# gabormarko/3D-semantic-segmentation

Hardware: AMD Instinct MI355X
Metric: Mvoxel-views/sec (higher is better)
Workload: dtype f32; 1 GPU; R2: 200000 voxels x 300 views x 968x548x512 fp32 feature maps, room-shell scene seed 0, dmin 0.01 dmax 10 step 0.5*voxel; views_per_call=60, resident_feature_maps=60, parallelism=single GPU

## Files before the change

3d-semantic-segmentation_amd/csrc/voxproj.hip:

```cpp
#include <hip/hip_runtime.h>

#include <cmath>
#include <cstdarg>
#include <cstdint>
#include <cstdio>
#include <cstdlib>
#include <cstring>
#include <algorithm>
#include <chrono>
#include <mutex>
#include <unordered_map>
#include <vector>

#include "voxproj.h"

#include "vp_common.h"
#include "vp_tables.h"
#include "vp_march.h"
#include "vp_gather.h"
#include "vp_aux.h"
#include "vp_prep.h"
#include "vp_aggregate.h"
#include "vp_render.h"
#include "vp_query.h"
// ... 199 lines not shown
        long long ppx = rec.opt_part_px > 0 ? rec.opt_part_px : std::max<long long>(1, heavy_t);
        ppx = std::max(ppx, (px2 + l.slot_cap - 1) / l.slot_cap);
        plan.part_px = (int)std::min<long long>(ppx, 2147483647ll);
        heavy_t = std::max(heavy_t, plan.part_px);
        plan.heavy_t = plan.part_t = heavy_t;
    } else if (one_split) {
        const long long T = rec.opt_one_view_split > 0 ? rec.opt_one_view_split : rec.opt_heavy_t > 0 ? rec.opt_heavy_t : 0;
        long long ppx = rec.opt_part_px > 0 ? std::max(rec.opt_part_px, (px2 + l.slot_cap - 1) / l.slot_cap) : 0;
        if (ppx == 0 && T > 0) ppx = std::max<long long>((T + ONE_VIEW_T_RATIO - 1) / ONE_VIEW_T_RATIO, (px2 + l.slot_cap - 1) / l.slot_cap);
        plan.part_px = (int)std::min<long long>(ppx, 2147483646ll);
        plan.dyn_px_min = ppx > 0 ? 0 : ONE_VIEW_PART_MIN;
        plan.heavy_t = plan.part_t = T > 0 ? (int)std::min<long long>(std::max(T, ppx), 2147483646ll) : 0;
        plan.dyn_t_ratio = T > 0 ? 0 : ONE_VIEW_T_RATIO;
        plan.dyn_t_floor = (long long)H * W <= GATHER_G32_SMALL_IMAGE ? ONE_VIEW_T_FLOOR_SMALL : 0;
        plan.cell_in_item = 1;
        heavy_t = plan.heavy_t;
    } else if (one_view) {
        plan.count_heavy = 0;
    }
    static_assert(sizeof(PlanArgs) == sizeof(int) * 8, "PlanArgs is kept as ints in the workspace record");
    if (gather_only) { memcpy(&plan, st->last_plan, sizeof(plan)); heavy_t = plan.heavy_t; }
    const int part_px = plan.part_px;
    const bool plans_parts = part_px > 0 || plan.dyn_px_min > 0;
#ifdef VP_DIAG
    if (flags & VP_FLAG_DIAG_EVALS) heavy_t = -1;
    if (flags & VP_FLAG_DIAG_WAVES) heavy_t = -2;
#endif
    const int wl_blocks = (int)((n_rows + 256 * WL_PER_THREAD - 1) / (256 * WL_PER_THREAD));
    int4 *parts = (int4 *)(ws + l.parts[q]), *split = (int4 *)(ws + l.split[q]), *pmeta = (int4 *)(ws + l.pmeta[q]);
    float *prow = (float *)(ws + l.prow[q]);
    int *hit_waves = (int *)(ws + l.hitcnt[q]);
#define VP_LAUNCH_WORKLIST(STREAM)                                                                                              \
    hipLaunchKernelGGL(k_worklist, dim3((unsigned)(wl_blocks + (B * V + 255) / 256)), dim3(256), 0, STREAM, (const int *)cnt_call,   \
                       plan, (long long)n_rows, work, status, wl_blocks, vmi, viewtab, B * V, row_lo, row_hi, parts, split, \
                       (int)l.slot_cap, rec.sticky_dev, (const int *)cell_of_id, (const int *)hit_waves, (int)l.n_hitcnt)
    if (gather_only) {
        VP_HIP(hipMemsetAsync(status + ST_WORK0, 0, ST_PLAN_WORDS * sizeof(int), s0));
        VP_LAUNCH_WORKLIST(s0);
    }
    if (!gather_only) {
        ProfSpan sp; sp.begin(0, s1);
        hipLaunchKernelGGL(k_zero_call, dim3((unsigned)((n_rows + 1023) / 1024)), dim3(256), 0, s1, status, cnt_call, (long long)n_rows,
                           status0, rec.sticky_dev, WS_MAGIC, rec.gen, expect_tables, hit_waves,
                           (plan.dyn_px_min > 0 && !march_only) ? l.n_hitcnt : 0ll);
        sp.end();
    }
    if (!gather_only) {
        FirstHitArgs fa;
        fa.occ = (const long long *)occ; fa.vmi = vmi; fa.intr = intr; fa.near2 = near2; fa.dist = dist;
        fa.nby = l.nby; fa.nbx = l.nbx; fa.nblk = l.nblk; fa.hit = march_only ? (int *)ids_out : hit; fa.cnt_call = cnt_call;
        fa.heavy_list = heavy_list; fa.heavy_t = ((one_view && !one_split) || heavy_t < 0) ? heavy_t : 2147483647;
        fa.hit_waves = (plan.dyn_px_min > 0 && l.n_hitcnt > 0) ? hit_waves : nullptr;
        if (march_only) { fa.heavy_t = 2147483647; fa.hit_waves = nullptr; }
        fa.status = status; fa.sticky = rec.sticky_dev;
        const dim3 grid((W + 15) / 16, (H + 15) / 16, B * V);
        ProfSpan sp; sp.begin(1, s1);
        if (flags & VP_FLAG_EXACT_MARCH) {
            hipLaunchKernelGGL(k_first_hit<0>, grid, dim3(256), 0, s1, fa, p);
        } else {
            bool beside_gather = false;
            if (pipe && ps->used[q ^ 1]) {
                beside_gather = hipEventQuery(ps->call_done[q ^ 1]) == hipErrorNotReady;
                (void)hipGetLastError();
            }
            const size_t row_bytes = size_t(C) * (feats_f16 ? 2 : 4);
            size_t lds_req = beside_gather ? (row_bytes <= 1024 ? 30 : 41) * 1024 : 0;
            if (rec.opt_march_lds_kb >= 0) lds_req = size_t(std::min<long long>(rec.opt_march_lds_kb, 64)) * 1024;
            hipLaunchKernelGGL(k_first_hit<1>, grid, dim3(256), lds_req, s1, fa, p);
        }
        if (!march_only) VP_LAUNCH_WORKLIST(s1);
        sp.end();
    }
    if (march_only) {
        VP_HIP(hipGetLastError());
        ps->last_q = 0;
        if (flags & VP_FLAG_SYNC) return workspace_status_impl(workspace, stream_, true);
        return VP_OK;
    }
    if (pipe && !gather_only) VP_HIP(hipEventRecord(ps->fh_done[q], s1));

    GatherArgs g;
    g.feats = feats; g.hit = hit; g.viewtab = viewtab; g.intr = intr; g.cell_of_id = cell_of_id;
    g.cnt_call = cnt_call; g.heavy_list = heavy_list; g.n_heavy = status + ST_NHEAVY;
    g.row_lo = (int)row_lo; g.row_hi = (int)row_hi;
    g.work = work; g.work_n = status + ST_WORK0;
    g.parts = parts; g.split = split; g.pmeta = pmeta; g.prow = prow;
    g.host_word = nullptr; g.host_seq = 0;
    g.parts_on = (one_view && plans_parts) ? 1 : 0; g.slot_cap = (int)l.slot_cap; g.count = count; g.views_hit = views_hit; g.out = out; g.status = status;
    const int vec_ok = feats_f16 ? 2 : ((C % 4 == 0) && (((uintptr_t)feats & 15) == 0) && (((uintptr_t)out & 15) == 0)) ? 1 : 0;
    const bool small_image = (long long)B * V >= 8 && (long long)H * W <= GATHER_G32_SMALL_IMAGE;
    g.heavy_blocks = 0;
    if (pipe && !gather_only) VP_HIP(hipStreamWaitEvent(s0, ps->fh_done[q], 0));
    if (one_view) {
        ProfSpan sp; sp.begin(2, s0);
        const int per_cu = rec.opt_one_view > 0 ? (int)std::min<long long>(rec.opt_one_view, 256) : 16;
        const long long want = rec.opt_one_view >= 1000 ? rec.opt_one_view - 1000 : (long long)device_cus() * per_cu;
        const long long cap = (n_rows - 1 + 3) / 4;
        const unsigned nblk = (unsigned)std::max<long long>(1, std::min(want, cap));
        g.heavy_blocks = (heavy_t != 2147483647 && !plans_parts) ? (int)nblk : 0;
        volatile int *note = nullptr;
        if ((flags & VP_FLAG_SYNC) && plans_parts && n_rows > 1) {
            rec.split_seq = (rec.split_seq + 1) & 0x7fffu;
            note = rec.sticky_host + ST_HOST_NSPLIT;
            *note = 0;
            g.host_word = rec.sticky_dev + ST_HOST_NSPLIT; g.host_seq = (int)rec.split_seq;
        }
        if (n_rows > 1) VP_DISPATCH_GATHER_ONE((long long)H * W <= GATHER_G32_SMALL_IMAGE, vec_ok, C, dim3(nblk), dim3(256), 0, s0, g, p);
        sp.end();
        bool combine = n_rows > 1 && plans_parts;
        if (combine && note) {
            const auto t0 = std::chrono::steady_clock::now();
            for (unsigned spin = 0;; spin++) {
                const unsigned v = (unsigned)*note;
                if ((v >> 31) && ((v >> 16) & 0x7fffu) == rec.split_seq) { combine = (v & 0xffffu) != 0; break; }
                if ((spin & 63) == 63 && std::chrono::steady_clock::now() - t0 > std::chrono::milliseconds(2)) break;
                __builtin_ia32_pause();
            }
        }
        if (combine) {
            ProfSpan sc; sc.begin(3, s0);
// ... 820 lines not shown
    if (radius > 0)
        if (int rc = eval_check_workspace(workspace, workspace_bytes, W, H)) return rc;
    hipStream_t stream = (hipStream_t)stream_;
    const long long n = (long long)W * H;
    unsigned char *pband = nullptr, *tband = nullptr;
    if (radius > 0) {
        const size_t plane = align256((size_t)n);
        pband = (unsigned char *)workspace;
        tband = pband + plane;
        unsigned char *ok = tband + plane;
        eval_launch_band((const int *)pred, W, H, radius, pband, ok, stream);
        eval_launch_band((const int *)target, W, H, radius, tband, ok, stream);
    }
    const dim3 grid((unsigned)std::min<long long>((n + 255) / 256, EVAL_SCORE_BLOCKS));
#define VP_EVAL_SCORES(LDS) hipLaunchKernelGGL((k_eval_scores<LDS>), grid, dim3(256), 0, stream, (const int *)pred, (const int *)target, n, \
        P, (const unsigned char *)pband, (const unsigned char *)tband, (unsigned long long *)confusion,                              \
        (unsigned long long *)skipped, (unsigned long long *)bnd_inter, (unsigned long long *)bnd_union)
    if (P <= EVAL_LDS_P) VP_EVAL_SCORES(true); else VP_EVAL_SCORES(false);
#undef VP_EVAL_SCORES
    VP_HIP(hipGetLastError());
    return VP_OK;
}

long long vp_workspace_table_builds(const void *workspace)
{
    WsState *rec = ws_state(workspace, false);
    return rec ? rec->builds : 0;
}

int vp_workspace_create(void *workspace, size_t workspace_bytes)
{
    if (!workspace) return fail(VP_EINVAL, "null workspace");
    if ((uintptr_t)workspace & 255) return fail(VP_EWORKSPACE, "workspace must be 256-byte aligned");
    if (workspace_bytes < 2 * align256(ST_WORDS * sizeof(int))) return fail(VP_EWORKSPACE, "workspace has %zu bytes, need at least %zu", workspace_bytes, 2 * align256(ST_WORDS * sizeof(int)));
    ws_forget(workspace);
    (void)ws_state(workspace, true);
    return VP_OK;
}

int vp_workspace_set_option(void *workspace, int option, long long value)
{
    if (!workspace) return fail(VP_EINVAL, "null workspace");
    WsState *rec = ws_state(workspace, true);
    switch (option) {
    case VP_OPT_HEAVY_THRESHOLD: rec->opt_heavy_t = value > 0 ? value : -1; return VP_OK;
    case VP_OPT_MARCH_LDS_KB:
        if (value > 64) return fail(VP_EINVAL, "VP_OPT_MARCH_LDS_KB = %lld: the march's dynamic-LDS reservation is limited to 64 KiB (0 .. 64; < 0 = default)", value);
        rec->opt_march_lds_kb = value >= 0 ? value : -1; return VP_OK;
    case VP_OPT_ROW_BEGIN:       rec->opt_row_begin = value >= 0 ? value : -1; return VP_OK;
    case VP_OPT_ROW_END:         rec->opt_row_end = value >= 0 ? value : -1; return VP_OK;
    case VP_OPT_ONE_VIEW_GATHER: rec->opt_one_view = value >= 0 ? value : -1; return VP_OK;
    case VP_OPT_PART_PIXELS:     rec->opt_part_px = value > 0 ? value : -1; return VP_OK;
    case VP_OPT_ONE_VIEW_SPLIT:  rec->opt_one_view_split = value >= 0 ? value : -1; return VP_OK;
    default: return fail(VP_EINVAL, "unknown workspace option %d", option);
    }
}

int vp_workspace_release(void *workspace)
{
    ws_forget(workspace);
    return VP_OK;
}

}
```

3d-semantic-segmentation_amd/csrc/vp_common.h:

```cpp
#pragma once

namespace {

thread_local char g_err[512] = "";

int fail(int code, const char *fmt, ...)
{
    va_list ap;
    va_start(ap, fmt);
    vsnprintf(g_err, sizeof(g_err), fmt, ap);
    va_end(ap);
    return code;
}

#define VP_HIP(call)                                                                      \
    do {                                                                                  \
        hipError_t e_ = (call);                                                           \
        if (e_ != hipSuccess)                                                             \
            return fail(VP_EHIP, "%s failed: %s (%s:%d)", #call, hipGetErrorString(e_),   \
                        __FILE__, __LINE__);                                              \
    } while (0)

struct Profile {
    std::mutex mu;
// ... 6 lines not shown
        if (used * 2 == pool.size()) {
            hipEvent_t e0, e1;
            if (hipEventCreate(&e0) != hipSuccess || hipEventCreate(&e1) != hipSuccess) return -1;
            pool.push_back(e0); pool.push_back(e1); kind.push_back(0);
        }
        kind[used] = k;
        return (int)used++;
    }
} g_prof;

struct ProfSpan {
    int idx = -1;
    hipStream_t stream = nullptr;
    void begin(int k, hipStream_t s)
    {
        std::lock_guard<std::mutex> g(g_prof.mu);
        if (!g_prof.on) return;
        idx = g_prof.next(k);
        stream = s;
        if (idx >= 0) (void)hipEventRecord(g_prof.pool[idx * 2], s);
    }
    void end()
    {
        if (idx < 0) return;
        std::lock_guard<std::mutex> g(g_prof.mu);
        (void)hipEventRecord(g_prof.pool[idx * 2 + 1], stream);
        idx = -1;
    }
};

struct PipeState {
    hipStream_t side = nullptr;
    hipEvent_t fh_done[2] = {nullptr, nullptr};
    hipEvent_t call_done[2] = {nullptr, nullptr};
    bool used[2] = {false, false};
    long long calls = 0;
    int last_q = 0;
    bool ok = false;
};
struct WsState {
    unsigned gen = 0;
    int B = 0, dimz = 0, dimy = 0, dimx = 0;
    long long n_rows = 0;
    bool copy_valid = false;
    long long builds = 0;
    bool opened = false;
    int *sticky_host = nullptr, *sticky_dev = nullptr;
    long long opt_heavy_t = -1;
    long long opt_march_lds_kb = -1;
    long long opt_row_begin = -1, opt_row_end = -1;
    long long opt_one_view = -1;
    long long opt_part_px = -1;
    long long opt_one_view_split = -1;
    int last_B = 0, last_V = 0, last_H = 0, last_W = 0, last_C = 0, last_q = 0;
    bool last_f16 = false, last_ranged = false;
    int last_plan[8] = {0, 0, 0, 0, 0, 0, 0, 0};
    unsigned split_seq = 0;
    const void *last_feats = nullptr, *last_out = nullptr, *last_count = nullptr, *last_vmi = nullptr;
    bool has_hit = false;
    size_t hit_off = 0;
    PipeState pipe;
};
std::mutex g_ws_mu;
std::unordered_map<const void *, WsState *> g_ws;
unsigned g_next_gen = 0;

WsState *ws_state(const void *workspace, bool create)
{
    std::lock_guard<std::mutex> g(g_ws_mu);
    auto it = g_ws.find(workspace);
    if (it != g_ws.end()) return it->second;
    if (!create) return nullptr;
    if (g_next_gen == 0) g_next_gen = (unsigned)std::chrono::steady_clock::now().time_since_epoch().count() | 1u;
    WsState *st = new WsState();
    st->gen = g_next_gen;
    g_next_gen += 2;
    g_ws.emplace(workspace, st);
    return st;
}

void pipe_destroy(PipeState &ps)
{
    if (!ps.ok) return;
    (void)hipStreamSynchronize(ps.side);
    (void)hipStreamDestroy(ps.side);
    for (int q = 0; q < 2; q++) {
        (void)hipEventDestroy(ps.fh_done[q]);
        (void)hipEventDestroy(ps.call_done[q]);
    }
    ps = PipeState();
}

void ws_forget(const void *workspace)
{
    WsState *st = nullptr;
    {
        std::lock_guard<std::mutex> g(g_ws_mu);
        auto it = g_ws.find(workspace);
        if (it == g_ws.end()) return;
        st = it->second;
        g_ws.erase(it);
    }
    pipe_destroy(st->pipe);
    if (st->sticky_host) (void)hipHostFree(st->sticky_host);
    delete st;
}
// ... 42 lines not shown
    int width, height;
    float dmin, dmax, inc;
    float ox, oy, oz, vs;
    int dimz, dimy, dimx;
    int B, V, C;
    long long n_rows;
};

enum { ST_BADID = 0, ST_BOXMISS = 1, ST_NHEAVY = 2, ST_ZERO = 3 , ST_STUCK = 4, ST_OCCDIFF = 5, ST_STALE = 6,
       ST_HEAVY_T = 7,
       ST_NHIT = 8,
       ST_PART_T = 9, ST_PART_PX = 10,
       ST_WORK0 = 16, WORK_CLASSES = 8,
       ST_NPARTS = 24, ST_NSPLIT = 25,
       ST_PLAN_WORDS = WORK_CLASSES + 2,
       ST_CALL_WORDS = 32,
       ST_HDR_MAGIC = 56, ST_HDR_GEN = 57, ST_HDR_TABLES = 58,
       ST_HOST_NSPLIT = 60,
       ST_STICKY_STALE = 61, ST_STICKY_BADID = 62, ST_STICKY_STUCK = 63, ST_WORDS = 64 };
constexpr unsigned WS_MAGIC = 0x56585033u;
#ifdef VP_DIAG
enum { VP_FLAG_DIAG_EVALS = 1 << 20,
       VP_FLAG_DIAG_WAVES = 1 << 21 };
#endif

inline unsigned tables_key(int B, int dimz, int dimy, int dimx, long long n_rows, long long builds)
{
    unsigned long long h = 0x9E3779B97F4A7C15ull;
    const long long v[6] = {B, dimz, dimy, dimx, n_rows, builds};
    for (long long x : v) { h ^= (unsigned long long)x + 0x9E3779B97F4A7C15ull + (h << 6) + (h >> 2); h *= 0xff51afd7ed558ccdull; }
    const unsigned k = (unsigned)(h ^ (h >> 32));
    return k ? k : 1u;
}

struct __attribute__((aligned(32))) NearRec {
    unsigned long long p0, p1, p2;
    unsigned long long dist;
};

struct ViewEntry {
    float inv[9];
    float pos[3];
    float ok;
    float pad[3];
};

struct Layout {
    size_t cell_of_id, mask64, near2, dist, dist_tmp;
    size_t occ_copy;
    size_t status[2], cnt_call[2], heavy[2], work[2], viewtab[2], hit[2];
    size_t parts[2], split[2], pmeta[2], prow[2];
    size_t hitcnt[2];
    long long n_hitcnt;
    long long slot_cap;
    size_t total;
    int nbx, nby, nbz;
    long long nblk;
};

inline size_t align256(size_t v) { return (v + 255) & ~size_t(255); }

#ifndef VP_MAX_SLOTS
#define VP_MAX_SLOTS 65536
#endif
#ifndef VP_ONE_VIEW_SLOTS
#define VP_ONE_VIEW_SLOTS 8192
#endif
inline long long part_slot_cap(int B, int V, int H, int W, int C)
{
    const long long px2 = 2ll * B * V * (long long)H * W;
    const long long by_bytes = std::max<long long>(1024, ((long long)VP_MAX_SLOTS * 2048) / (std::max(C, 1) * 4ll));
    long long cap = std::max<long long>(64, std::min<long long>(VP_MAX_SLOTS, std::min(px2, by_bytes)));
    if ((long long)B * V == 1) cap = std::min<long long>(cap, VP_ONE_VIEW_SLOTS);
    return cap;
}

Layout make_layout(int B, int V, int H, int W, int C, long long n_rows, int dimz, int dimy, int dimx, size_t capacity = 0)
{
    Layout l;
    size_t off = 0;
    l.nbx = (dimx + 3) / 4; l.nby = (dimy + 3) / 4; l.nbz = (dimz + 3) / 4;
    l.nblk = ((long long)l.nbx * l.nby * l.nbz + 15) & ~15ll;
    l.status[0] = off;   off += align256(ST_WORDS * sizeof(int));
    l.status[1] = off;   off += align256(ST_WORDS * sizeof(int));
    l.cell_of_id = off;  off += align256(size_t(B) * size_t(n_rows) * sizeof(int));
    l.mask64 = off;      off += align256(size_t(B) * l.nblk * sizeof(unsigned long long));
    l.near2 = off;       off += align256(size_t(B) * l.nblk * sizeof(NearRec));
    l.dist = off;        off += align256(size_t(B) * l.nblk);
    l.dist_tmp = off;    off += align256(size_t(B) * l.nblk);
    l.occ_copy = off;    off += align256(size_t(B) * size_t(dimz) * dimy * dimx * sizeof(int));
    for (int q = 0; q < 2; q++) {
        l.cnt_call[q] = off; off += align256(size_t(n_rows) * sizeof(int));
        l.heavy[q] = off;    off += align256(size_t(n_rows) * sizeof(int));
        l.work[q] = off;     off += align256(size_t(WORK_CLASSES) * size_t(n_rows) * sizeof(int));
    }
    l.slot_cap = part_slot_cap(B, V, H, W, C);
    const size_t sz_view = align256(size_t(B) * V * sizeof(ViewEntry)), sz_hit = align256(size_t(B) * V * H * W * sizeof(int));
    const size_t sz_i4 = align256(size_t(l.slot_cap) * 16), sz_prow = align256(size_t(l.slot_cap) * size_t(C) * sizeof(float));
    l.n_hitcnt = (long long)B * V == 1 ? (long long)((W + 15) / 16) * ((H + 15) / 16) * 4 : 0;
    const size_t sz_hc = align256(size_t(l.n_hitcnt) * sizeof(int));
    const size_t per_set = sz_view + sz_hit + 3 * sz_i4 + sz_prow + sz_hc;
    size_t half = per_set;
    if (capacity > off + 2 * per_set) half = ((capacity - off) / 2) & ~size_t(255);
    for (int q = 0; q < 2; q++) {
        l.viewtab[q] = off + q * half;
        l.hit[q] = l.viewtab[q] + sz_view;
        l.parts[q] = l.hit[q] + sz_hit;
        l.split[q] = l.parts[q] + sz_i4;
        l.pmeta[q] = l.split[q] + sz_i4;
        l.prow[q] = l.pmeta[q] + sz_i4;
        l.hitcnt[q] = l.prow[q] + sz_prow;
    }
    l.total = off + 2 * per_set;
    return l;
}

}
```

3d-semantic-segmentation_amd/csrc/vp_march.h:

```cpp
#pragma once

namespace {

struct FirstHitArgs {
    const long long *occ;
    const float *vmi;
    const float *intr;
    const NearRec *near2;
    const unsigned char *dist;
    int nby, nbx;
    long long nblk;
    int *hit;
    int *cnt_call;
    int *heavy_list;
    int heavy_t;
    int *hit_waves;
    int *status;
    int *sticky;
};

struct MarchView {
    const long long *occ_b;
    const NearRec *near_b;
    const unsigned char *dist_b;
    int nby, nbx;
    float cpx, cpy, cpz;
    float fx, fy, mx, my, fw, fh;
    float rvs;
};

struct MarchRay {
    float cdx, cdy, cdz;
    float wdx, wdy, wdz;
    float tEnd;
    float inv_dcell;
    float thr;
    bool leap_ok;
};

struct MarchBlock {
    unsigned cur_blk = 0xffffffffu;
    int cur_d = 0;
    unsigned long long p0 = 0ull, p1 = 0ull, p2 = 0ull;
};

struct MarchBinade {
    float bT2 = 0.0f, bTu = 0.0f, bg = 0.0f, brg = 0.0f;
};

__device__ __forceinline__ int march_sample(const Params &p, const MarchView &mv, const MarchRay &r, MarchBlock &mb, float t, int &D)
{
    const float px = mv.cpx + t * r.wdx, py = mv.cpy + t * r.wdy, pz = mv.cpz + t * r.wdz;
    const float ax = px - p.ox, ay = py - p.oy, az = pz - p.oz;
    const float qx = ax * mv.rvs, qy = ay * mv.rvs, qz = az * mv.rvs;
    const float rx = rintf(qx), ry = rintf(qy), rz = rintf(qz);
    const bool safe = (fabsf(qx - rx) < r.thr) & (fabsf(qy - ry) < r.thr) & (fabsf(qz - rz) < r.thr);
    int ix = (int)rx, iy = (int)ry, iz = (int)rz;
    if (__builtin_expect(!safe, 0)) {
        ix = f2i_sat(round_half_away(ax / p.vs));
        iy = f2i_sat(round_half_away(ay / p.vs));
        iz = f2i_sat(round_half_away(az / p.vs));
    }
    D = 0;
    const bool ing = ((unsigned)ix < (unsigned)p.dimx) & ((unsigned)iy < (unsigned)p.dimy) & ((unsigned)iz < (unsigned)p.dimz);
    if (__builtin_expect(ing, 1)) {
        const unsigned blk = ((unsigned)(iz >> 2) * (unsigned)mv.nby + (unsigned)(iy >> 2)) * (unsigned)mv.nbx + (unsigned)(ix >> 2);
        if (blk != mb.cur_blk) {
            mb.cur_blk = blk;
            const NearRec n3 = mv.near_b[blk];
// ... 88 lines not shown
    const float cpz = m[8] * 0.0f + m[9] * 0.0f + m[10] * 0.0f + m[11] * 1.0f;
    float wx = m[0] * cdx + m[1] * cdy + m[2] * cdz + m[3] * 0.0f;
    float wy = m[4] * cdx + m[5] * cdy + m[6] * cdz + m[7] * 0.0f;
    float wz = m[8] * cdx + m[9] * cdy + m[10] * cdz + m[11] * 0.0f;
    inv = 1.0f / sqrtf(wx * wx + wy * wy + wz * wz);
    const float wdx = wx * inv, wdy = wy * inv, wdz = wz * inv;

    const float d2r = 1.0f / cdz;
    float t = d2r * p.dmin;
    const float tEnd = d2r * p.dmax;
    const long long cells = (long long)p.dimz * p.dimy * p.dimx;
    const long long *occ_b = occ + (long long)b * cells;
    const float fw = (float)p.width, fh = (float)p.height;
    int id = 0;
    if ((t < tEnd) && !(tEnd + p.inc > tEnd)) {
        atomicOr(&status[ST_STUCK], 1);
        *(volatile int *)&fa.sticky[ST_STICKY_STUCK] = 1;
        t = tEnd;
    }
    if constexpr (!ACCEL) {
        while (t < tEnd) {
            const float px = cpx + t * wdx, py = cpy + t * wdy, pz = cpz + t * wdz;
            const int ix = f2i_sat(round_half_away((px - p.ox) / p.vs));
            const int iy = f2i_sat(round_half_away((py - p.oy) / p.vs));
            const int iz = f2i_sat(round_half_away((pz - p.oz) / p.vs));
            const float camx = cdx * t, camy = cdy * t, camz = cdz * t;
            const float u = fx * (camx / camz) + mx;
            const float v = fy * (camy / camz) + my;
            const bool inb = (u >= 0.0f) && (u < fw) && (v >= 0.0f) && (v < fh);
            if (inb && ix >= 0 && iy >= 0 && iz >= 0 && ix < p.dimx && iy < p.dimy && iz < p.dimz) {
                id = (int)occ_b[((long long)iz * p.dimy + iy) * p.dimx + ix];
                if (id != 0) break;
            }
            t += p.inc;
        }
    } else {
        MarchView mv;
        mv.occ_b = occ_b;
        mv.near_b = fa.near2 + (long long)b * nblk;
        mv.dist_b = fa.dist + (long long)b * nblk;
        mv.nby = fa.nby; mv.nbx = fa.nbx;
        mv.cpx = cpx; mv.cpy = cpy; mv.cpz = cpz;
        mv.fx = fx; mv.fy = fy; mv.mx = mx; mv.my = my; mv.fw = fw; mv.fh = fh;
        mv.rvs = 1.0f / p.vs;
        MarchRay r;
        r.cdx = cdx; r.cdy = cdy; r.cdz = cdz; r.wdx = wdx; r.wdy = wdy; r.wdz = wdz; r.tEnd = tEnd;
        const float dcell = fabsf(p.inc * mv.rvs) * fmaxf(fabsf(wdx), fmaxf(fabsf(wdy), fabsf(wdz))) * 1.01f + 1e-6f;
        const float span = (fabsf(cpx) + fabsf(cpy) + fabsf(cpz) + fabsf(p.ox) + fabsf(p.oy) + fabsf(p.oz) + fabsf(tEnd)) * fabsf(mv.rvs);
        r.leap_ok = (span < 131072.0f) & (fabsf(tEnd) < 1.0e5f * fabsf(p.inc)) & (dcell == dcell) & (dcell < 1.0e6f);
        r.inv_dcell = r.leap_ok ? 0.999f / dcell : 0.0f;
        r.thr = r.leap_ok ? 0.5f - span * 0x1p-21f : -1.0f;
        MarchBlock mb;
        MarchBinade bn;
#ifdef VP_DIAG
        int dbg_leap = 0, dbg_fine = 0;
#endif
        while (t < tEnd) {
            int D;
            id = march_sample(p, mv, r, mb, t, D);
            if (id != 0) break;
#ifdef VP_DIAG
            if (heavy_t < 0) { if (D >= 2) dbg_leap++; else dbg_fine++; }
            dbg_it++;
#endif
            march_advance(p.inc, tEnd, bn, t, march_steps(r, D));
        }
#ifdef VP_DIAG
        if (heavy_t == -2) {
            const unsigned long long t1 = __builtin_amdgcn_s_memrealtime();
            const int l = threadIdx.x & 63;
            const int mine = dbg_leap + dbg_fine;
            for (int off = 32; off > 0; off >>= 1) dbg_it = max(dbg_it, __shfl_xor(dbg_it, off));
            hit[((long long)bv * p.height + y) * p.width + x] = l == 0 ? (int)(unsigned)dbg_t0 : l == 1 ? (int)(unsigned)t1 : l == 2 ? dbg_it : mine;
            return;
        }
        if (heavy_t < 0) {
            hit[((long long)bv * p.height + y) * p.width + x] = (min(dbg_leap, 1023) << 10) | min(dbg_fine, 1023);
            return;
        }
#endif
    }
    if (id != 0 && (id < 0 || id >= p.n_rows)) {
        atomicOr(&status[ST_BADID], 1);
        *(volatile int *)&fa.sticky[ST_STICKY_BADID] = 1;
        id = 0;
    }
    hit[((long long)bv * p.height + y) * p.width + x] = id;
    {
        const int lane_ = threadIdx.x & 63;
        int my_n = 0;
        unsigned long long todo = __ballot(id != 0);
        if (fa.hit_waves && todo != 0ull && lane_ == __builtin_ctzll(todo))
            fa.hit_waves[((long long)blockIdx.y * gridDim.x + blockIdx.x) * 4 + (threadIdx.x >> 6)] = __popcll(todo);
        while (todo) {
            const int l = __builtin_ctzll(todo);
            const int cur = __builtin_amdgcn_readlane(id, l);
            const unsigned long long m = __ballot(id == cur);
            if (lane_ == l) my_n = __popcll(m);
            todo &= ~m;
        }
        if (my_n > 0) {
            const int old = atomicAdd(&cnt_call[id], my_n);
            if (old <= heavy_t && old + my_n > heavy_t) heavy_list[atomicAdd(&status[ST_NHEAVY], 1)] = id;
        }
    }
}

template <int MODE>
__global__ __launch_bounds__(256) void k_first_hit(FirstHitArgs fa, Params p)
{
    const int wave = threadIdx.x >> 6, lane = threadIdx.x & 63;
    const int x = blockIdx.x * 16 + (wave & 1) * 8 + (lane & 7);
    const int y = blockIdx.y * 16 + (wave >> 1) * 8 + (lane >> 3);
    first_hit_body<MODE>(fa, p, x, y, blockIdx.z);
}

}
```

3d-semantic-segmentation_amd/voxproj_host.py:

```python
import collections
import ctypes
import os
import subprocess
import threading
import weakref

_HERE = os.path.dirname(os.path.abspath(__file__))
LIB_PATH = os.environ.get("VOXPROJ_LIB") or os.path.join(_HERE, "libvoxproj.so")

VP_OK = 0
VP_FLAG_SYNC = 1
VP_FLAG_REUSE_ACCEL = 2
VP_FLAG_EXACT_MARCH = 4
VP_FLAG_PIPELINE = 8
VP_FLAG_VERIFY_ACCEL = 16
VP_FLAG_SERIAL_SUMS = 32
VP_FLAG_GATHER_ONLY = 64

_lib = None
_lock = threading.Lock()

EXACT_MARCH = False
ACCEL_CACHE = True
_default_options = {}
_options_version = 0


def set_default_option(option, value):
    global _options_version
    if value is None:
        _default_options.pop(int(option), None)
    else:
        _default_options[int(option)] = int(value)
    _options_version += 1

EXPORTS = [
    "vp_abi_version", "vp_last_error", "vp_workspace_bytes", "vp_project_features",
    "vp_workspace_status", "vp_workspace_counters", "vp_copy_hit_image",
    "vp_profile_enable", "vp_profile_read", "vp_workspace_release", "vp_project_colors",
    "vp_project_features_f16", "vp_nearest_voxel",
    "vp_stream_read", "vp_workspace_table_builds", "vp_colors_workspace_bytes",
    "vp_upsample_workspace_bytes", "vp_upsample_features", "vp_voxel_coords", "vp_scatter_occupancy",
    "vp_aggregate_view_f16", "vp_workspace_create", "vp_workspace_set_option",
    "vp_first_hit_ids", "vp_render_features", "vp_query_workspace_bytes", "vp_query_features",
    "vp_splat_workspace_bytes", "vp_splat_project", "vp_splat_rasterize",
    "vp_splat_backward_workspace_bytes", "vp_splat_rasterize_backward",
    "vp_splat_geometry_backward_workspace_bytes", "vp_splat_rasterize_backward_geometry",
    "vp_splat_loss_workspace_bytes", "vp_splat_rasterize_loss", "vp_splat_loss_backward",
    "vp_label_scores_workspace_bytes", "vp_label_boundary", "vp_label_scores",
]
VP_ABI_VERSION = 4
VP_OPT_HEAVY_THRESHOLD = 1
VP_OPT_MARCH_LDS_KB = 2
VP_OPT_ROW_BEGIN = 3
VP_OPT_ROW_END = 4
VP_OPT_ONE_VIEW_GATHER = 5
VP_OPT_PART_PIXELS = 6
VP_OPT_ONE_VIEW_SPLIT = 7
VP_LOSS_SUM = 0
VP_LOSS_MEAN = 1


class VoxprojError(RuntimeError):
    pass


def build(force=False):
    csrc = os.path.join(_HERE, "csrc")
    srcs = [os.path.join(csrc, f) for f in os.listdir(csrc) if f == "voxproj.hip" or (f.startswith("vp_") and f.endswith(".h"))]
    srcs.append(os.path.join(os.path.dirname(_HERE), "include", "voxproj.h"))
    newest = max(os.path.getmtime(f) for f in srcs)
    if force or not os.path.exists(LIB_PATH) or os.path.getmtime(LIB_PATH) < newest:
        subprocess.check_call(["make", "-C", os.path.join(_HERE, "csrc"), "-s"] + (["-B"] if force else []))
    return LIB_PATH


def ext_path():
    import sysconfig
    return os.path.join(_HERE, "project_features_cuda" + sysconfig.get_config_var("EXT_SUFFIX"))


def build_ext(force=False):
    import sys
    build(force)
    out = ext_path()
    src = os.path.join(_HERE, "csrc", "project_features_ext.cpp")
    hdr = os.path.join(os.path.dirname(_HERE), "include", "voxproj.h")
    newest = max(os.path.getmtime(src), os.path.getmtime(hdr), os.path.getmtime(os.path.join(_HERE, "setup.py")))
    if not force and os.path.exists(out) and os.path.getmtime(out) >= newest:
        return out
    subprocess.check_call([sys.executable, "setup.py", "-q", "build_ext", "--inplace"] + (["--force"] if force else []), cwd=_HERE)
    return out


def lib():
    global _lib
    with _lock:
        if _lib is None:
            if not os.path.exists(LIB_PATH):
                raise VoxprojError(
                    f"{LIB_PATH} is missing: build it with `make -C {os.path.join(_HERE, 'csrc')}` "
                    "(there is no CPU fallback)")
            L = ctypes.CDLL(LIB_PATH)
            L.vp_abi_version.restype = ctypes.c_int
            L.vp_last_error.restype = ctypes.c_char_p
            L.vp_workspace_bytes.restype = ctypes.c_size_t
            L.vp_workspace_bytes.argtypes = [ctypes.c_int] * 8 + [ctypes.c_int64]
            vp = ctypes.c_void_p
            L.vp_project_features.restype = ctypes.c_int
            L.vp_project_features.argtypes = [
                vp, vp, vp, vp, ctypes.POINTER(ctypes.c_float), vp, vp, vp, ctypes.POINTER(ctypes.c_float),
# ... 83 lines not shown
                [ctypes.c_size_t, vp, ctypes.c_size_t, vp]
            L.vp_label_scores_workspace_bytes.restype = ctypes.c_size_t
            L.vp_label_scores_workspace_bytes.argtypes = [ctypes.c_int, ctypes.c_int]
            L.vp_label_boundary.restype = ctypes.c_int
            L.vp_label_boundary.argtypes = [vp, ctypes.c_int, ctypes.c_int, ctypes.c_int, vp, vp, ctypes.c_size_t, vp]
            L.vp_label_scores.restype = ctypes.c_int
            L.vp_label_scores.argtypes = [vp, vp] + [ctypes.c_int] * 4 + [vp] * 5 + [ctypes.c_size_t, vp]
            if L.vp_abi_version() != VP_ABI_VERSION:
                raise VoxprojError(f"{LIB_PATH} has ABI version {L.vp_abi_version()}, this package needs {VP_ABI_VERSION}: rebuild it")
            _lib = L
    return _lib


def last_error():
    return lib().vp_last_error().decode("utf-8", "replace")


def check(rc):
    if rc != VP_OK:
        raise VoxprojError(f"voxproj error {rc}: {last_error()}")


def workspace_bytes(B, V, H, W, C, dimz, dimy, dimx, n_rows):
    return int(lib().vp_workspace_bytes(B, V, H, W, C, dimz, dimy, dimx, n_rows))


class Workspace:

    def __init__(self):
        self.buf = None
        self.accel_key = None
        self.options = {}
        self._applied = None

    def ensure(self, nbytes, device):
        import torch
        if self.buf is None or self.buf.numel() < nbytes + 256 or self.buf.device != device:
            if self.buf is not None:
                import torch as _t
                check(lib().vp_workspace_status(self.ptr(), _t.cuda.current_stream(self.buf.device).cuda_stream))
            self.release()
            self.buf = torch.empty(int(nbytes) + 256, dtype=torch.uint8, device=device)
            self.accel_key = None
            check(lib().vp_workspace_create(self.ptr(), self.capacity()))
            self._applied = None
        self._push_options()
        return self.ptr()

    def _push_options(self):
        state = (_options_version, tuple(sorted(self.options.items())))
        if self.buf is None or self._applied == state:
            return
        merged = {VP_OPT_HEAVY_THRESHOLD: -1, VP_OPT_MARCH_LDS_KB: -1, VP_OPT_ROW_BEGIN: -1, VP_OPT_ROW_END: -1, VP_OPT_ONE_VIEW_GATHER: -1,
                  VP_OPT_PART_PIXELS: -1, VP_OPT_ONE_VIEW_SPLIT: -1}
        merged.update(_default_options)
        merged.update(self.options)
        for opt, val in merged.items():
            check(lib().vp_workspace_set_option(self.ptr(), int(opt), int(val)))
        self._applied = state

    def set_option(self, option, value):
        if value is None:
            self.options.pop(int(option), None)
        else:
            self.options[int(option)] = int(value)
        self._push_options()

    def set_row_range(self, begin=None, end=None):
        self.set_option(VP_OPT_ROW_BEGIN, begin)
        self.set_option(VP_OPT_ROW_END, end)

    def ptr(self):
        return (self.buf.data_ptr() + 255) & ~255

    def capacity(self):
        return self.buf.numel() - (self.ptr() - self.buf.data_ptr())

    def release(self):
        if self.buf is not None and _lib is not None:
            _lib.vp_workspace_release(self.ptr())

    def __del__(self):
        try:
            self.release()
        except Exception:
            pass


_workspaces = {}


def get_workspace(device):
    key = (device.type, device.index)
    ws = _workspaces.get(key)
    if ws is None:
        ws = _workspaces[key] = Workspace()
    return ws


def project_features_raw(feats, occ, vmi, intr, opts5, count, out, grid_origin3, voxel_size,
                         workspace=None, sync=True, reuse_accel=None, exact_march=None, pipeline=False,
                         views_hit=None, verify_accel=False, gather_only=False, serial_sums=False, extra_flags=0):
    import torch
    B, V, H, W, C = feats.shape
    _, dimz, dimy, dimx = occ.shape
    n_rows = int(count.shape[0])
    ws = workspace if workspace is not None else get_workspace(feats.device)
# ... 797 lines not shown
```

include/voxproj.h:

```cpp
#ifndef VOXPROJ_H
#define VOXPROJ_H

#include <stddef.h>
#include <stdint.h>

#ifdef __cplusplus
extern "C" {
#endif

#define VP_ABI_VERSION 4

enum {
    VP_OK = 0,
    VP_EINVAL = -1,
    VP_EWORKSPACE = -2,
    VP_EHIP = -3,
    VP_EBADID = -4,
    VP_EUNSUPPORTED = -5
};

enum {
    VP_FLAG_SYNC = 1,
    VP_FLAG_REUSE_ACCEL = 2,
    VP_FLAG_EXACT_MARCH = 4,
// ... 15 lines not shown
                        const float *grid_origin_host, float voxel_size,
                        int B, int V, int H, int W, int C,
                        int dimz, int dimy, int dimx, int64_t n_rows,
                        void *workspace, size_t workspace_bytes,
                        void *stream, int flags);

int vp_nearest_voxel(const float *pts_sorted, const int32_t *perm, const int32_t *cell_start,
                     const double *grid_origin3, double cell_size, int nx, int ny, int nz,
                     const float *queries, int64_t M, int64_t *out, void *stream);

int vp_stream_read(const float *src, int64_t n_floats, float *sink, void *stream);

int vp_project_features_f16(const void *feats_f16, const int64_t *occ, const float *vmi,
                            const float *intr, const float *opts_host,
                            int32_t *count, float *out, int32_t *views_hit,
                            const float *grid_origin_host, float voxel_size,
                            int B, int V, int H, int W, int C,
                            int dimz, int dimy, int dimx, int64_t n_rows,
                            void *workspace, size_t workspace_bytes,
                            void *stream, int flags);

int vp_workspace_status(void *workspace, void *stream);

int vp_workspace_counters(void *workspace, int32_t *host_words, int n, void *stream);

int vp_profile_enable(int on);
int vp_profile_read(double *ms4, int64_t *launches4);

size_t vp_colors_workspace_bytes(int64_t n_rows);
int vp_project_colors(const int32_t *occ, int dimz, int dimy, int dimx,
                      const float *c2w, const float *intr, int V,
                      const float *grid_origin_host, double voxel_size,
                      const uint8_t *images, int img_h, int img_w,
                      float *color_sum, int32_t *hit_count, int32_t *first_view, int32_t *pixel_uv,
                      int64_t n_rows, int view_base, void *workspace, size_t workspace_bytes, void *stream);

size_t vp_upsample_workspace_bytes(int C, int h, int w, int src_is_f16);
int vp_upsample_features(const void *src_chw, int src_is_f16, int C, int h, int w,
                         void *dst_hwc, int dst_is_f16, int H, int W,
                         void *workspace, size_t workspace_bytes, void *stream);

int vp_voxel_coords(const float *points_xyz, int64_t N, const float *grid_origin_host, float voxel_size,
                    int32_t *coords, int32_t *scratch8_dev, int32_t *minmax_host, void *stream);
int vp_scatter_occupancy(const int32_t *coords, int64_t N, const int32_t *shift3_host,
                         int dimz, int dimy, int dimx, int32_t *occ, int32_t *scratch8_dev, void *stream);

int vp_aggregate_view_f16(float *view_sum, int32_t *view_count, void *run16, int32_t *views, int32_t *first_view,
                          int view_index, int32_t *nonfinite_dev, int64_t n_rows, int C, void *stream);

int vp_workspace_create(void *workspace, size_t workspace_bytes);
int vp_workspace_release(void *workspace);

enum { VP_OPT_HEAVY_THRESHOLD = 1, VP_OPT_MARCH_LDS_KB = 2, VP_OPT_ROW_BEGIN = 3, VP_OPT_ROW_END = 4, VP_OPT_ONE_VIEW_GATHER = 5,
       VP_OPT_PART_PIXELS = 6, VP_OPT_ONE_VIEW_SPLIT = 7 };
int vp_workspace_set_option(void *workspace, int option, long long value);

long long vp_workspace_table_builds(const void *workspace);

int vp_copy_hit_image(const void *workspace, int32_t *dst, int B, int V, int H, int W,
                      int C, int dimz, int dimy, int dimx, int64_t n_rows, void *stream);

int vp_first_hit_ids(const int64_t *occ, const float *vmi, const float *intr, const float *opts_host,
                     const float *grid_origin_host, float voxel_size,
                     int B, int V, int H, int W, int dimz, int dimy, int dimx, int64_t n_rows,
                     int32_t *ids, void *workspace, size_t workspace_bytes, void *stream, int flags);
int vp_render_features(const int32_t *ids, int64_t n_pixels, const float *rows, int64_t n_rows, int C,
                       void *dst, int dst_is_f16, int32_t *bad_ids, void *stream);

size_t vp_query_workspace_bytes(int P, int C);
int vp_query_features(const void *rows, int rows_is_f16, int64_t n_rows, int C, int64_t row_stride, const float *text,
                      int P, float scale, float *logits, int32_t *labels, float *margin, int32_t *n_nonfinite,
                      void *workspace, size_t workspace_bytes, void *stream);

size_t vp_splat_workspace_bytes(int64_t n_gaussians, int W, int H, int64_t capacity);
int vp_splat_project(const float *means, const float *quats, const float *scales, const float *opacities,
                     int64_t n_gaussians, const float *viewmat, float fx, float fy, float cx, float cy, int W, int H,
                     float near_plane, float far_plane, float eps2d, int64_t *n_isect, int32_t *n_nonfinite,
                     void *workspace, size_t workspace_bytes, void *stream);
int vp_splat_rasterize(const float *features, int D, int64_t row_stride, int64_t n_gaussians, int W, int H,
                       int64_t capacity, int32_t *labels, float *confidence, float *alpha, float *logits,
                       int32_t *status, void *workspace, size_t workspace_bytes, void *stream);

size_t vp_splat_backward_workspace_bytes(int64_t capacity, int D);
int vp_splat_rasterize_backward(const float *features, int D, int64_t row_stride, int64_t n_gaussians, int W, int H,
                                int64_t capacity, const float *grad_logits, const float *grad_alpha,
                                float *grad_features, float *grad_opacities, int32_t *status, void *workspace,
                                size_t workspace_bytes, void *bwd_workspace, size_t bwd_bytes, void *stream);

size_t vp_splat_geometry_backward_workspace_bytes(int64_t capacity, int D);
int vp_splat_rasterize_backward_geometry(const float *means, const float *quats, const float *scales, const float *features,
                                         int D, int64_t row_stride, int64_t n_gaussians, const float *viewmat, float fx,
                                         float fy, float cx, float cy, int W, int H, float eps2d, int64_t capacity,
                                         const float *grad_logits, const float *grad_alpha, float *grad_means,
                                         float *grad_quats, float *grad_scales, float *grad_features, float *grad_opacities,
                                         float *grad_screen, int32_t *status, void *workspace, size_t workspace_bytes,
                                         void *bwd_workspace, size_t bwd_bytes, void *stream);

#define VP_LOSS_SUM 0
#define VP_LOSS_MEAN 1
size_t vp_splat_loss_workspace_bytes(int W, int H);
int vp_splat_rasterize_loss(const float *features, int D, int64_t row_stride, int64_t n_gaussians, int W, int H,
                            int64_t capacity, const int32_t *target, const float *pixel_weight, double *loss_stats,
                            float *pixel_loss, int32_t *labels, float *confidence, float *alpha, float *logits,
                            int32_t *status, void *workspace, size_t workspace_bytes, void *loss_workspace,
                            size_t loss_bytes, void *stream);
int vp_splat_loss_backward(const float *means, const float *quats, const float *scales, const float *features, int D,
                           int64_t row_stride, int64_t n_gaussians, const float *viewmat, float fx, float fy, float cx,
// ... 19 lines not shown
```

Measured before the change: 1149 Mvoxel-views/s.

## Precompute conservative per-wave march start steps with a tile prepass kernel

Adds a k_tile_start prepass that, for each 8x8-pixel wave tile, walks a conservative bounding cone through the distance field. It finds how many march steps every ray in the tile can safely skip before any possible hit. The first-hit kernel reads that per-wave count and advances its march before the per-ray loop, removing redundant empty-space stepping that is shared across a tile. It costs an extra kernel launch and workspace memory per call, and relies on conservative error bounds to keep results exact. It is on by default whenever B*V > 1.

```diff
diff --git a/3d-semantic-segmentation_amd/csrc/voxproj.hip b/3d-semantic-segmentation_amd/csrc/voxproj.hip
--- a/3d-semantic-segmentation_amd/csrc/voxproj.hip
+++ b/3d-semantic-segmentation_amd/csrc/voxproj.hip
@@ -275,7 +275,7 @@
         fa.heavy_list = heavy_list; fa.heavy_t = ((one_view && !one_split) || heavy_t < 0) ? heavy_t : 2147483647;
         fa.hit_waves = (plan.dyn_px_min > 0 && l.n_hitcnt > 0) ? hit_waves : nullptr;
         if (march_only) { fa.heavy_t = 2147483647; fa.hit_waves = nullptr; }
-        fa.status = status; fa.sticky = rec.sticky_dev;
+        fa.status = status; fa.sticky = rec.sticky_dev; fa.tile_start = nullptr;
         const dim3 grid((W + 15) / 16, (H + 15) / 16, B * V);
         ProfSpan sp; sp.begin(1, s1);
         if (flags & VP_FLAG_EXACT_MARCH) {
@@ -289,6 +289,15 @@
             const size_t row_bytes = size_t(C) * (feats_f16 ? 2 : 4);
             size_t lds_req = beside_gather ? (row_bytes <= 1024 ? 30 : 41) * 1024 : 0;
             if (rec.opt_march_lds_kb >= 0) lds_req = size_t(std::min<long long>(rec.opt_march_lds_kb, 64)) * 1024;
+            const bool tile_on = rec.opt_tile_start >= 0 ? rec.opt_tile_start != 0 : (long long)B * V > 1;
+            if (tile_on) {
+                TileStartArgs ta;
+                ta.vmi = vmi; ta.intr = intr; ta.near2 = near2; ta.dist = dist; ta.nby = l.nby; ta.nbx = l.nbx; ta.nblk = l.nblk;
+                ta.gx = (int)grid.x; ta.gy = (int)grid.y; ta.n_tiles = l.n_tiles;
+                ta.tile_start = (int *)(ws + l.tile_start[q]); ta.status = status;
+                hipLaunchKernelGGL(k_tile_start, dim3((unsigned)((l.n_tiles + 255) / 256)), dim3(256), 0, s1, ta, p);
+                fa.tile_start = ta.tile_start;
+            }
             hipLaunchKernelGGL(k_first_hit<1>, grid, dim3(256), lds_req, s1, fa, p);
         }
         if (!march_only) VP_LAUNCH_WORKLIST(s1);
@@ -1215,6 +1224,7 @@
     case VP_OPT_ONE_VIEW_GATHER: rec->opt_one_view = value >= 0 ? value : -1; return VP_OK;
     case VP_OPT_PART_PIXELS:     rec->opt_part_px = value > 0 ? value : -1; return VP_OK;
     case VP_OPT_ONE_VIEW_SPLIT:  rec->opt_one_view_split = value >= 0 ? value : -1; return VP_OK;
+    case VP_OPT_TILE_START:      rec->opt_tile_start = value >= 0 ? value : -1; return VP_OK;
     default: return fail(VP_EINVAL, "unknown workspace option %d", option);
     }
 }
diff --git a/3d-semantic-segmentation_amd/csrc/vp_common.h b/3d-semantic-segmentation_amd/csrc/vp_common.h
--- a/3d-semantic-segmentation_amd/csrc/vp_common.h
+++ b/3d-semantic-segmentation_amd/csrc/vp_common.h
@@ -82,6 +82,7 @@
     long long opt_one_view = -1;
     long long opt_part_px = -1;
     long long opt_one_view_split = -1;
+    long long opt_tile_start = -1;
     int last_B = 0, last_V = 0, last_H = 0, last_W = 0, last_C = 0, last_q = 0;
     bool last_f16 = false, last_ranged = false;
     int last_plan[8] = {0, 0, 0, 0, 0, 0, 0, 0};
@@ -230,6 +231,8 @@
     size_t parts[2], split[2], pmeta[2], prow[2];
     size_t hitcnt[2];
     long long n_hitcnt;
+    size_t tile_start[2];
+    long long n_tiles;
     long long slot_cap;
     size_t total;
     int nbx, nby, nbz;
@@ -277,7 +280,9 @@
     const size_t sz_i4 = align256(size_t(l.slot_cap) * 16), sz_prow = align256(size_t(l.slot_cap) * size_t(C) * sizeof(float));
     l.n_hitcnt = (long long)B * V == 1 ? (long long)((W + 15) / 16) * ((H + 15) / 16) * 4 : 0;
     const size_t sz_hc = align256(size_t(l.n_hitcnt) * sizeof(int));
-    const size_t per_set = sz_view + sz_hit + 3 * sz_i4 + sz_prow + sz_hc;
+    l.n_tiles = (long long)B * V * ((W + 15) / 16) * ((H + 15) / 16) * 4;
+    const size_t sz_ts = align256(size_t(l.n_tiles) * sizeof(int));
+    const size_t per_set = sz_view + sz_hit + 3 * sz_i4 + sz_prow + sz_hc + sz_ts;
     size_t half = per_set;
     if (capacity > off + 2 * per_set) half = ((capacity - off) / 2) & ~size_t(255);
     for (int q = 0; q < 2; q++) {
@@ -288,6 +293,7 @@
         l.pmeta[q] = l.split[q] + sz_i4;
         l.prow[q] = l.pmeta[q] + sz_i4;
         l.hitcnt[q] = l.prow[q] + sz_prow;
+        l.tile_start[q] = l.hitcnt[q] + sz_hc;
     }
     l.total = off + 2 * per_set;
     return l;
diff --git a/3d-semantic-segmentation_amd/csrc/vp_march.h b/3d-semantic-segmentation_amd/csrc/vp_march.h
--- a/3d-semantic-segmentation_amd/csrc/vp_march.h
+++ b/3d-semantic-segmentation_amd/csrc/vp_march.h
@@ -15,6 +15,7 @@
     int *heavy_list;
     int heavy_t;
     int *hit_waves;
+    const int *tile_start;
     int *status;
     int *sticky;
 };
@@ -209,6 +210,11 @@
         r.thr = r.leap_ok ? 0.5f - span * 0x1p-21f : -1.0f;
         MarchBlock mb;
         MarchBinade bn;
+        if (fa.tile_start) {
+            const int wave_u = __builtin_amdgcn_readfirstlane((int)(threadIdx.x >> 6));
+            const int J = fa.tile_start[(((long long)bv * gridDim.y + blockIdx.y) * gridDim.x + blockIdx.x) * 4 + wave_u];
+            if (J > 0 && t < tEnd) march_advance(p.inc, tEnd, bn, t, J);
+        }
 #ifdef VP_DIAG
         int dbg_leap = 0, dbg_fine = 0;
 #endif
@@ -263,6 +269,125 @@
     }
 }
 
+struct TileStartArgs {
+    const float *vmi;
+    const float *intr;
+    const NearRec *near2;
+    const unsigned char *dist;
+    int nby, nbx;
+    long long nblk;
+    int gx, gy;
+    long long n_tiles;
+    int *tile_start;
+    const int *status;
+};
+
+struct TileRay {
+    float vx, vy, vz;
+    float cdz;
+    float wx, wy, wz;
+};
+
+__device__ __forceinline__ TileRay tile_ray(const float *m, float fx, float fy, float mx, float my, float depth, float xp, float yp)
+{
+    TileRay r;
+    r.vx = depth * ((xp - mx) / fx); r.vy = depth * ((yp - my) / fy); r.vz = depth;
+    float inv = 1.0f / sqrtf(r.vx * r.vx + r.vy * r.vy + r.vz * r.vz);
+    const float cdx = r.vx * inv, cdy = r.vy * inv, cdz = r.vz * inv;
+    r.cdz = cdz;
+    const float wx = m[0] * cdx + m[1] * cdy + m[2] * cdz;
+    const float wy = m[4] * cdx + m[5] * cdy + m[6] * cdz;
+    const float wz = m[8] * cdx + m[9] * cdy + m[10] * cdz;
+    inv = 1.0f / sqrtf(wx * wx + wy * wy + wz * wz);
+    r.wx = wx * inv; r.wy = wy * inv; r.wz = wz * inv;
+    return r;
+}
+
+__device__ __forceinline__ int tile_bound(const Params &p, const TileStartArgs &ta, const NearRec *near_b, const unsigned char *dist_b,
+                                          int ix, int iy, int iz)
+{
+    const bool ing = ((unsigned)ix < (unsigned)p.dimx) & ((unsigned)iy < (unsigned)p.dimy) & ((unsigned)iz < (unsigned)p.dimz);
+    if (ing) {
+        const unsigned blk = ((unsigned)(iz >> 2) * (unsigned)ta.nby + (unsigned)(iy >> 2)) * (unsigned)ta.nbx + (unsigned)(ix >> 2);
+        const int dd = dist_b[blk];
+        if (dd >= 2) return (dd - 1) * 4 + 1;
+        const NearRec n3 = near_b[blk];
+        const int bit = ((iz & 3) << 4) | ((iy & 3) << 2) | (ix & 3);
+        return (int)((n3.p0 >> bit) & 1ull) | ((int)((n3.p1 >> bit) & 1ull) << 1) | ((int)((n3.p2 >> bit) & 1ull) << 2);
+    }
+    const int ex = ix < 0 ? -ix : (ix >= p.dimx ? ix - p.dimx + 1 : 0);
+    const int ey = iy < 0 ? -iy : (iy >= p.dimy ? iy - p.dimy + 1 : 0);
+    const int ez = iz < 0 ? -iz : (iz >= p.dimz ? iz - p.dimz + 1 : 0);
+    const int dbox = max(ex, max(ey, ez));
+    const int kx = min(max(ix, 0), p.dimx - 1), ky = min(max(iy, 0), p.dimy - 1), kz = min(max(iz, 0), p.dimz - 1);
+    const int dd = dist_b[((kz >> 2) * ta.nby + (ky >> 2)) * ta.nbx + (kx >> 2)];
+    const int din = dd > 0 ? (dd - 1) * 4 + 1 : 0;
+    return max(dbox, din - dbox);
+}
+
+constexpr int TILE_START_MAX = 1 << 24;
+constexpr int TILE_START_ITERS = 128;
+
+__device__ __forceinline__ int tile_start_steps(const TileStartArgs &ta, const Params &p, long long i)
+{
+    const int wave = (int)(i & 3);
+    const long long wg = i >> 2;
+    const int bx = (int)(wg % ta.gx), by = (int)((wg / ta.gx) % ta.gy), bv = (int)(wg / ((long long)ta.gx * ta.gy));
+    const int b = bv / p.V;
+    const float x0 = (float)(bx * 16 + (wave & 1) * 8), y0 = (float)(by * 16 + (wave >> 1) * 8);
+    const float *m = ta.vmi + (long long)bv * 16;
+    const float fx = ta.intr[b * 4 + 0], fy = ta.intr[b * 4 + 1], mx = ta.intr[b * 4 + 2], my = ta.intr[b * 4 + 3];
+    const float depth = 1.0f * (p.dmax - p.dmin) + p.dmin;
+    const TileRay c = tile_ray(m, fx, fy, mx, my, depth, x0 + 3.5f, y0 + 3.5f);
+    float dv = 0.0f, dw = 0.0f;
+    bool ok = true;
+    for (int k = 0; k < 4; k++) {
+        const TileRay r = tile_ray(m, fx, fy, mx, my, depth, x0 + (float)((k & 1) * 7), y0 + (float)((k >> 1) * 7));
+        const float ax = r.vx - c.vx, ay = r.vy - c.vy, az = r.vz - c.vz;
+        const float bx_ = r.wx - c.wx, by_ = r.wy - c.wy, bz_ = r.wz - c.wz;
+        const float a = sqrtf(ax * ax + ay * ay + az * az), bb = sqrtf(bx_ * bx_ + by_ * by_ + bz_ * bz_);
+        ok &= (a < 1.0e30f) & (bb < 0.5f);
+        dv = fmaxf(dv, a); dw = fmaxf(dw, bb);
+    }
+    const float cpx = m[3], cpy = m[7], cpz = m[11];
+    const float d2r = 1.0f / c.cdz;
+    const float t0 = d2r * p.dmin, tEnd = d2r * p.dmax;
+    dv = dv * 1.01f + sqrtf(c.vx * c.vx + c.vy * c.vy + c.vz * c.vz) * 1.0e-6f;
+    dw = dw * 1.01f + 1.0e-6f;
+    const float rdepth = 1.0f / fabsf(depth);
+    const float dt0 = fabsf(p.dmin) * rdepth * dv * 1.01f, dtE = fabsf(p.dmax) * rdepth * dv * 1.01f;
+    const float tmax = fmaxf(fabsf(t0), fabsf(tEnd)) + fmaxf(dt0, dtE) + p.inc;
+    const float rvs = 1.0f / p.vs, arvs = fabsf(rvs);
+    const float span = (fabsf(cpx) + fabsf(cpy) + fabsf(cpz) + fabsf(p.ox) + fabsf(p.oy) + fabsf(p.oz) + tmax) * arvs;
+    const float R0 = (dt0 * 1.001f + fabsf(t0) * dw) * arvs * 1.01f;
+    const float g = (tmax * 0x1p-24f * 1.02f + p.inc * dw) * arvs * 1.01f;
+    const float dcell = fabsf(p.inc * rvs) * fmaxf(fabsf(c.wx), fmaxf(fabsf(c.wy), fabsf(c.wz))) * 1.01f + 1e-6f;
+    ok &= (span < 131072.0f) & (tmax < 0.99e5f * p.inc) & (R0 < 1.0e6f) & (g < 1.0e6f) & (dcell < 1.0e6f) & (t0 < tEnd);
+    if (!ok) return 0;
+    const float inv_step = 0.999f / (dcell + g);
+    const NearRec *near_b = ta.near2 + (long long)b * ta.nblk;
+    const unsigned char *dist_b = ta.dist + (long long)b * ta.nblk;
+    int k = 0;
+    for (int it = 0; it < TILE_START_ITERS; it++) {
+        const float s = t0 + (float)k * p.inc;
+        if (!(s < tEnd)) break;
+        const float qx = ((cpx + s * c.wx) - p.ox) * rvs, qy = ((cpy + s * c.wy) - p.oy) * rvs, qz = ((cpz + s * c.wz) - p.oz) * rvs;
+        const int D = tile_bound(p, ta, near_b, dist_b, (int)rintf(qx), (int)rintf(qy), (int)rintf(qz));
+        const float room = (float)D - 1.75f - (R0 + (float)k * g);
+        if (!(room >= 0.0f)) break;
+        k += 1 + (int)fminf(room * inv_step, 4194304.0f);
+        if (k >= TILE_START_MAX) break;
+    }
+    return min(k, TILE_START_MAX);
+}
+
+__global__ __launch_bounds__(256) void k_tile_start(TileStartArgs ta, Params p)
+{
+    const long long i = (long long)blockIdx.x * 256 + threadIdx.x;
+    if (i >= ta.n_tiles) return;
+    ta.tile_start[i] = ta.status[ST_STALE] ? 0 : tile_start_steps(ta, p, i);
+}
+
 template <int MODE>
 __global__ __launch_bounds__(256) void k_first_hit(FirstHitArgs fa, Params p)
 {
diff --git a/3d-semantic-segmentation_amd/voxproj_host.py b/3d-semantic-segmentation_amd/voxproj_host.py
--- a/3d-semantic-segmentation_amd/voxproj_host.py
+++ b/3d-semantic-segmentation_amd/voxproj_host.py
@@ -57,6 +57,7 @@
 VP_OPT_ONE_VIEW_GATHER = 5
 VP_OPT_PART_PIXELS = 6
 VP_OPT_ONE_VIEW_SPLIT = 7
+VP_OPT_TILE_START = 8
 VP_LOSS_SUM = 0
 VP_LOSS_MEAN = 1
 
@@ -246,7 +247,7 @@
         if self.buf is None or self._applied == state:
             return
         merged = {VP_OPT_HEAVY_THRESHOLD: -1, VP_OPT_MARCH_LDS_KB: -1, VP_OPT_ROW_BEGIN: -1, VP_OPT_ROW_END: -1, VP_OPT_ONE_VIEW_GATHER: -1,
-                  VP_OPT_PART_PIXELS: -1, VP_OPT_ONE_VIEW_SPLIT: -1}
+                  VP_OPT_PART_PIXELS: -1, VP_OPT_ONE_VIEW_SPLIT: -1, VP_OPT_TILE_START: -1}
         merged.update(_default_options)
         merged.update(self.options)
         for opt, val in merged.items():
diff --git a/include/voxproj.h b/include/voxproj.h
--- a/include/voxproj.h
+++ b/include/voxproj.h
@@ -91,7 +91,7 @@
 int vp_workspace_release(void *workspace);
 
 enum { VP_OPT_HEAVY_THRESHOLD = 1, VP_OPT_MARCH_LDS_KB = 2, VP_OPT_ROW_BEGIN = 3, VP_OPT_ROW_END = 4, VP_OPT_ONE_VIEW_GATHER = 5,
-       VP_OPT_PART_PIXELS = 6, VP_OPT_ONE_VIEW_SPLIT = 7 };
+       VP_OPT_PART_PIXELS = 6, VP_OPT_ONE_VIEW_SPLIT = 7, VP_OPT_TILE_START = 8 };
 int vp_workspace_set_option(void *workspace, int option, long long value);
 
 long long vp_workspace_table_builds(const void *workspace);
```

Result: no change. 1151 Mvoxel-views/s, median of 2 (+0.2%).
